# facebookresearch/GPU-DPF

Measured on AMD Instinct MI355X. Metric: DPFs/sec, higher is better.
Workload: dtype int32; 1 GPU; model=dpf-pir, entries=1048576, entry_size=16, prf=AES128, batch_per_gpu=512, global_batch=512, parallelism=dp1-replicated

## Files before the change

csrc/hip/dpf_hip_api.h:

```cpp
#pragma once
#include <cstddef>
#include <cstdint>

namespace gpudpf_hip {

void launch_fused(std::uintptr_t keys, std::uintptr_t table, std::uintptr_t out,
                  std::uintptr_t aes_tabs, int batch, long long n, int depth,
                  int zlog, int prf, std::uintptr_t stream,
                  std::uintptr_t scratch = 0, std::size_t scratch_bytes = 0,
                  int entry_words = 16);
std::size_t eval_scratch_bytes(int batch, int depth, int zlog);

void launch_fused_binned(std::uintptr_t keys, std::uintptr_t table,
                         std::uintptr_t bins, std::uintptr_t out,
                         std::uintptr_t aes_tabs, int batch, long long n,
                         int depth, int zlog, long long num_bins, int prf,
                         std::uintptr_t stream, std::uintptr_t scratch = 0,
                         std::size_t scratch_bytes = 0, int entry_words = 16);

int eval_slog(int batch, int depth, int zlog);
int eval_units_per_wg(int prf, int n_units, int entry_words = 16);

void launch_expand(std::uintptr_t keys, std::uintptr_t out,
                   std::uintptr_t aes_tabs, int batch, long long n, int depth,
                   int zlog, int prf, std::uintptr_t stream,
                   std::uintptr_t scratch = 0, std::size_t scratch_bytes = 0);

void launch_bfs(std::uintptr_t keys, std::uintptr_t out,
                std::uintptr_t aes_tabs, int batch, long long n, int depth,
                int prf, std::uintptr_t stream);

void launch_coop(std::uintptr_t keys, std::uintptr_t table, std::uintptr_t out,
                 std::uintptr_t aes_tabs, long long n, int depth, int zlog,
                 int prf, bool fused, std::uintptr_t stream);

void launch_naive(std::uintptr_t keys, std::uintptr_t out,
                  std::uintptr_t aes_tabs, int batch, long long n, int depth,
                  int prf, std::uintptr_t stream);

void launch_prf_sol(std::uintptr_t aes_tabs, std::uintptr_t out, int blocks,
                    int iters, int prf, std::uintptr_t stream);

void launch_probe_alu(std::uintptr_t a, std::uintptr_t b,
                      std::uintptr_t add_out, std::uintptr_t mul_out,
                      int count, std::uintptr_t stream);
void launch_probe_prf(std::uintptr_t seeds, std::uintptr_t aes_tabs,
                      std::uintptr_t pair0, std::uintptr_t pair1,
                      std::uintptr_t single0, std::uintptr_t single1,
                      std::uintptr_t low0, std::uintptr_t low1, int count,
                      int prf, std::uintptr_t stream);

struct KSplit;

KSplit gemm128_split(long long M, long long N, long long K);
void launch_gemm128(std::uintptr_t a, std::uintptr_t bt, std::uintptr_t c,
                    std::uintptr_t partials, std::size_t partials_bytes,
                    long long M, long long N, long long K,
                    std::uintptr_t stream);

KSplit gemm_u32_split(long long M, long long N, long long K);
void launch_digits(std::uintptr_t in, std::uintptr_t out, long long count,
                   std::uintptr_t stream);
void launch_gemm_u32_mfma(std::uintptr_t da, std::uintptr_t dbt,
                          std::uintptr_t c, long long M, long long N,
                          long long K, std::uintptr_t stream);

KSplit gemm_u32_stream_split(int batch, long long K, long long N);
void launch_gemm_u32_stream(std::uintptr_t a, std::uintptr_t b,
                            std::uintptr_t c, int batch, long long K,
                            long long N, std::uintptr_t stream);

}
```

csrc/hip/dpf_probes.hip:

```cpp

#include <hip/hip_runtime.h>

#include "dpf_hip_api.h"
#include "hip_util.h"
#include "prf_device.h"

namespace gpudpf_hip {

template <int PRF>
__global__ __launch_bounds__(PRF == PRF_AES128 ? 1024 : 256) void prf_sol_kernel(
    const u32* __restrict__ aes_tabs, u32* __restrict__ out, int iters) {
  extern __shared__ u32 smem[];
  const AesLds T = aes_lds_init<PRF>(smem, aes_tabs);
  uint4 seed = make_uint4(threadIdx.x + 1, blockIdx.x + 2, 3, 4);
  for (int i = 0; i < iters; ++i) {
    uint4 r0, r1;
    prf_pair<PRF>(seed, T, r0, r1);
    seed = make_uint4(r0.x ^ r1.x, r0.y ^ r1.y, r0.z ^ r1.z, r0.w ^ r1.w);
  }
  out[(u64)blockIdx.x * blockDim.x + threadIdx.x] = seed.x;
}

void launch_prf_sol(std::uintptr_t aes_tabs, std::uintptr_t out, int blocks,
                    int iters, int prf, std::uintptr_t stream) {
  const size_t shmem = aes_lds_u32(prf) * sizeof(u32);
  with_prf(prf, [&](auto P) {
    constexpr int PRF = decltype(P)::value;
    allow_large_lds((const void*)prf_sol_kernel<PRF>, shmem);
    const bool wide = PRF == PRF_AES128 && blocks % 4 == 0;
    hipLaunchKernelGGL(prf_sol_kernel<PRF>, dim3(wide ? blocks / 4 : blocks),
                       dim3(wide ? 1024 : 256), shmem, as_stream(stream),
                       as_ptr<const u32>(aes_tabs), as_ptr<u32>(out), iters);
  });
  HIP_CHECK(hipGetLastError());
}

__global__ __launch_bounds__(256) void probe_alu_kernel(
    const uint4* __restrict__ a, const uint4* __restrict__ b,
    uint4* __restrict__ add_out, uint4* __restrict__ mul_out, int count) {
  const int i = (int)(blockIdx.x * blockDim.x + threadIdx.x);
  if (i >= count) return;
  add_out[i] = add128(a[i], b[i]);
  const unsigned __int128 x =
      ((unsigned __int128)(((u64)a[i].w << 32) | a[i].z) << 64) |
      (((u64)a[i].y << 32) | a[i].x);
  const unsigned __int128 y =
      ((unsigned __int128)(((u64)b[i].w << 32) | b[i].z) << 64) |
      (((u64)b[i].y << 32) | b[i].x);
  const unsigned __int128 r = x * y;
  const u64 lo = (u64)r, hi = (u64)(r >> 64);
  mul_out[i] = make_uint4((u32)lo, (u32)(lo >> 32), (u32)hi, (u32)(hi >> 32));
}

template <int PRF>
__global__ __launch_bounds__(256) void probe_prf_kernel(
    const uint4* __restrict__ seeds, const u32* __restrict__ aes_tabs,
    uint4* __restrict__ pair0, uint4* __restrict__ pair1,
    uint4* __restrict__ single0, uint4* __restrict__ single1,
    u32* __restrict__ low0, u32* __restrict__ low1, int count) {
  extern __shared__ u32 smem[];
  const AesLds T = aes_lds_init<PRF>(smem, aes_tabs);
  const int i = (int)(blockIdx.x * blockDim.x + threadIdx.x);
  if (i >= count) return;
  const uint4 s = seeds[i];
  uint4 r0, r1;
  prf_pair<PRF>(s, T, r0, r1);
  pair0[i] = r0;
  pair1[i] = r1;
  single0[i] = prf_full<PRF>(s, 0, T);
  single1[i] = prf_full<PRF>(s, 1, T);
  u32 l0, l1;
  prf_pair_low<PRF>(s, T, l0, l1);
  low0[i] = l0;
  low1[i] = l1;
}

void launch_probe_alu(std::uintptr_t a, std::uintptr_t b,
                      std::uintptr_t add_out, std::uintptr_t mul_out,
                      int count, std::uintptr_t stream) {
  const int blocks = (count + 255) / 256;
  hipLaunchKernelGGL(probe_alu_kernel, dim3(blocks), dim3(256), 0,
                     as_stream(stream), as_ptr<const uint4>(a),
                     as_ptr<const uint4>(b), as_ptr<uint4>(add_out),
                     as_ptr<uint4>(mul_out), count);
  HIP_CHECK(hipGetLastError());
}

void launch_probe_prf(std::uintptr_t seeds, std::uintptr_t aes_tabs,
                      std::uintptr_t pair0, std::uintptr_t pair1,
                      std::uintptr_t single0, std::uintptr_t single1,
                      std::uintptr_t low0, std::uintptr_t low1, int count,
                      int prf, std::uintptr_t stream) {
  const int blocks = (count + 255) / 256;
  const size_t shmem = aes_lds_u32(prf) * sizeof(u32);
  with_prf(prf, [&](auto P) {
    constexpr int PRF = decltype(P)::value;
    allow_large_lds((const void*)probe_prf_kernel<PRF>, shmem);
    hipLaunchKernelGGL(probe_prf_kernel<PRF>, dim3(blocks), dim3(256), shmem,
                       as_stream(stream), as_ptr<const uint4>(seeds),
                       as_ptr<const u32>(aes_tabs), as_ptr<uint4>(pair0),
                       as_ptr<uint4>(pair1), as_ptr<uint4>(single0),
                       as_ptr<uint4>(single1), as_ptr<u32>(low0),
                       as_ptr<u32>(low1), count);
  });
  HIP_CHECK(hipGetLastError());
}

}
```

csrc/hip/hip_bindings.cc:

```cpp

#include <hip/hip_runtime.h>
#include <pybind11/pybind11.h>
#include <pybind11/stl.h>

#include <map>
#include <mutex>

#include "dpf_core.h"
#include "dpf_hip_api.h"
#include "hip_util.h"

namespace py = pybind11;

namespace {

std::mutex g_aes_mu;
std::map<int, void*> g_aes_tables;

std::uintptr_t ensure_aes_tables(int device) {
  std::lock_guard<std::mutex> lock(g_aes_mu);
  auto it = g_aes_tables.find(device);
  if (it != g_aes_tables.end()) return reinterpret_cast<std::uintptr_t>(it->second);
  gpudpf::u32 host[5 * 256];
  gpudpf::aes128_tables(host, host + 256, host + 512, host + 768, host + 1024);
  int prev = 0;
  HIP_CHECK(hipGetDevice(&prev));
  HIP_CHECK(hipSetDevice(device));
  void* dev = nullptr;
  HIP_CHECK(hipMalloc(&dev, sizeof(host)));
  HIP_CHECK(hipMemcpy(dev, host, sizeof(host), hipMemcpyHostToDevice));
  HIP_CHECK(hipSetDevice(prev));
  g_aes_tables[device] = dev;
  return reinterpret_cast<std::uintptr_t>(dev);
}

int device_count() {
  int n = 0;
  hipError_t e = hipGetDeviceCount(&n);
  if (e != hipSuccess) return 0;
  return n;
}

template <class... A>
auto split_tuple(gpudpf_hip::KSplit (*query)(A...)) {
  return [query](A... args) {
    const gpudpf_hip::KSplit s = query(args...);
    return std::make_pair(s.segs, s.kchunk);
  };
}

}

PYBIND11_MODULE(_hip, m) {
  m.doc() = "gpudpf MI355X HIP kernels (gfx950)";
  m.def("eval_fused", &gpudpf_hip::launch_fused, py::arg("keys"),
        py::arg("table"), py::arg("out"), py::arg("aes_tabs"), py::arg("batch"),
        py::arg("n"), py::arg("depth"), py::arg("zlog"), py::arg("prf"),
        py::arg("stream"), py::arg("scratch") = 0,
        py::arg("scratch_bytes") = 0, py::arg("entry_words") = 16,
        py::call_guard<py::gil_scoped_release>());
  m.def("eval_fused_binned", &gpudpf_hip::launch_fused_binned,
        py::arg("keys"), py::arg("table"), py::arg("bins"), py::arg("out"),
        py::arg("aes_tabs"), py::arg("batch"), py::arg("n"), py::arg("depth"),
        py::arg("zlog"), py::arg("num_bins"), py::arg("prf"),
        py::arg("stream"), py::arg("scratch") = 0,
        py::arg("scratch_bytes") = 0, py::arg("entry_words") = 16,
        py::call_guard<py::gil_scoped_release>());
  m.def("eval_scratch_bytes", &gpudpf_hip::eval_scratch_bytes,
        py::arg("batch"), py::arg("depth"), py::arg("zlog"));
  m.def("eval_slog", &gpudpf_hip::eval_slog, py::arg("batch"),
        py::arg("depth"), py::arg("zlog"));
  m.def("eval_units_per_wg", &gpudpf_hip::eval_units_per_wg, py::arg("prf"),
        py::arg("n_units"), py::arg("entry_words") = 16);
  m.def("eval_expand", &gpudpf_hip::launch_expand, py::arg("keys"),
        py::arg("out"), py::arg("aes_tabs"), py::arg("batch"), py::arg("n"),
        py::arg("depth"), py::arg("zlog"), py::arg("prf"), py::arg("stream"),
        py::arg("scratch") = 0, py::arg("scratch_bytes") = 0,
        py::call_guard<py::gil_scoped_release>());
  m.def("eval_bfs", &gpudpf_hip::launch_bfs, py::arg("keys"), py::arg("out"),
        py::arg("aes_tabs"), py::arg("batch"), py::arg("n"), py::arg("depth"),
        py::arg("prf"), py::arg("stream"),
        py::call_guard<py::gil_scoped_release>());
  m.def("eval_coop", &gpudpf_hip::launch_coop, py::arg("keys"),
        py::arg("table"), py::arg("out"), py::arg("aes_tabs"), py::arg("n"),
        py::arg("depth"), py::arg("zlog"), py::arg("prf"), py::arg("fused"),
        py::arg("stream"), py::call_guard<py::gil_scoped_release>());
  m.def("eval_naive", &gpudpf_hip::launch_naive, py::arg("keys"),
        py::arg("out"), py::arg("aes_tabs"), py::arg("batch"), py::arg("n"),
        py::arg("depth"), py::arg("prf"), py::arg("stream"),
        py::call_guard<py::gil_scoped_release>());
  m.def("gemm128", &gpudpf_hip::launch_gemm128, py::arg("a"), py::arg("bt"),
        py::arg("c"), py::arg("partials"), py::arg("partials_bytes"),
        py::arg("m"), py::arg("n"), py::arg("k"), py::arg("stream"),
        py::call_guard<py::gil_scoped_release>());
  m.def("gemm128_split", split_tuple(&gpudpf_hip::gemm128_split),
        py::arg("m"), py::arg("n"), py::arg("k"));
  m.def("prf_sol", &gpudpf_hip::launch_prf_sol, py::arg("aes_tabs"),
        py::arg("out"), py::arg("blocks"), py::arg("iters"), py::arg("prf"),
        py::arg("stream"), py::call_guard<py::gil_scoped_release>());
  m.def("digits", &gpudpf_hip::launch_digits, py::arg("inp"), py::arg("out"),
        py::arg("count"), py::arg("stream"),
        py::call_guard<py::gil_scoped_release>());
  m.def("gemm_u32_mfma", &gpudpf_hip::launch_gemm_u32_mfma, py::arg("da"),
        py::arg("dbt"), py::arg("c"), py::arg("m"), py::arg("n"), py::arg("k"),
        py::arg("stream"), py::call_guard<py::gil_scoped_release>());
  m.def("gemm_u32_split", split_tuple(&gpudpf_hip::gemm_u32_split),
        py::arg("m"), py::arg("n"), py::arg("k"));
  m.def("gemm_u32_stream", &gpudpf_hip::launch_gemm_u32_stream, py::arg("a"),
        py::arg("b"), py::arg("c"), py::arg("batch"), py::arg("k"),
        py::arg("n"), py::arg("stream"),
        py::call_guard<py::gil_scoped_release>());
  m.def("gemm_u32_stream_split",
        split_tuple(&gpudpf_hip::gemm_u32_stream_split), py::arg("batch"),
        py::arg("k"), py::arg("n"));
  m.def("probe_alu", &gpudpf_hip::launch_probe_alu, py::arg("a"), py::arg("b"),
        py::arg("add_out"), py::arg("mul_out"), py::arg("count"),
        py::arg("stream"), py::call_guard<py::gil_scoped_release>());
  m.def("probe_prf", &gpudpf_hip::launch_probe_prf, py::arg("seeds"),
        py::arg("aes_tabs"), py::arg("pair0"), py::arg("pair1"),
        py::arg("single0"), py::arg("single1"), py::arg("low0"),
        py::arg("low1"), py::arg("count"), py::arg("prf"), py::arg("stream"),
        py::call_guard<py::gil_scoped_release>());
  m.def("ensure_aes_tables", &ensure_aes_tables, py::arg("device"));
  m.def("device_count", &device_count);
}
```

csrc/hip/prf_device.h:

```cpp
#pragma once
#include "hip_util.h"

namespace gpudpf_hip {

__device__ __forceinline__ uint4 add128(uint4 a, uint4 b) {
  u64 alo = ((u64)a.y << 32) | a.x, ahi = ((u64)a.w << 32) | a.z;
  u64 blo = ((u64)b.y << 32) | b.x, bhi = ((u64)b.w << 32) | b.z;
  u64 lo = alo + blo;
  u64 hi = ahi + bhi + (lo < alo ? 1u : 0u);
  return make_uint4((u32)lo, (u32)(lo >> 32), (u32)hi, (u32)(hi >> 32));
}

__device__ __forceinline__ u32 rotl(u32 v, int s) {
  return (v << s) | (v >> (32 - s));
}
__device__ __forceinline__ u32 rotr8(u32 v) { return (v >> 8) | (v << 24); }
__device__ __forceinline__ u32 rotr16(u32 v) { return (v >> 16) | (v << 16); }
__device__ __forceinline__ u32 rotr24(u32 v) { return (v >> 24) | (v << 8); }

__device__ __forceinline__ uint4 key_root(const int* key) {
  const int* rp = key + kKeyRootInt;
  return make_uint4((u32)rp[0], (u32)rp[1], (u32)rp[2], (u32)rp[3]);
}

__device__ __forceinline__ uint4 prf_dummy_full(uint4 seed, u32 pos) {
  unsigned __int128 s =
      ((unsigned __int128)(((u64)seed.w << 32) | seed.z) << 64) |
      (((u64)seed.y << 32) | seed.x);
  unsigned __int128 m = (unsigned __int128)(pos + 4242u);
  unsigned __int128 r = s * m + m;
  u64 lo = (u64)r, hi = (u64)(r >> 64);
  return make_uint4((u32)lo, (u32)(lo >> 32), (u32)hi, (u32)(hi >> 32));
}

template <int N>
__device__ __forceinline__ void stream_init(u32 (&x)[16][N], int pos_w,
                                            const u32 (&init)[16]) {
#pragma unroll
  for (int w = 0; w < 16; ++w)
#pragma unroll
    for (int i = 0; i < N; ++i) x[w][i] = init[w] + (w == pos_w ? i : 0);
}

template <int N>
__device__ __forceinline__ uint4 stream_out(const u32 (&x)[16][N], int i,
                                            int lo, uint4 seed) {
  return make_uint4(x[lo][i] + seed.x, x[lo - 1][i] + seed.y,
                    x[lo - 2][i] + seed.z, x[lo - 3][i] + seed.w);
}

template <int PART = 4, int N>
__device__ __forceinline__ void salsa_qr(u32 (&x)[16][N], int a, int b, int c,
                                         int d) {
  auto step = [&](int t, int p, int q, int s) {
#pragma unroll
    for (int i = 0; i < N; ++i) x[t][i] ^= rotl(x[p][i] + x[q][i], s);
  };
  step(b, a, d, 7);
  if constexpr (PART > 1) step(c, b, a, 9);
  if constexpr (PART > 2) step(d, c, b, 13);
  if constexpr (PART > 3) step(a, d, c, 18);
}

template <bool LOW, int N>
__device__ __forceinline__ void salsa12(uint4 seed, u32 pos, u32 (&x)[16][N]) {
  stream_init(x, 9, {0x65787061u, seed.w, seed.z, seed.y, seed.x, 0x6e642033u,
                     0, 0, 0, pos, 0x322d6279u, 0, 0, 0, 0, 0x7465206bu});
#pragma unroll
  for (int r = 0; r < (LOW ? 5 : 6); ++r) {
    salsa_qr(x, 0, 4, 8, 12);
    salsa_qr(x, 5, 9, 13, 1);
    salsa_qr(x, 10, 14, 2, 6);
    salsa_qr(x, 15, 3, 7, 11);
    salsa_qr(x, 0, 1, 2, 3);
    salsa_qr(x, 5, 6, 7, 4);
    salsa_qr(x, 10, 11, 8, 9);
    salsa_qr(x, 15, 12, 13, 14);
  }
  if constexpr (LOW) {
    salsa_qr<1>(x, 0, 4, 8, 12);
    salsa_qr(x, 5, 9, 13, 1);
    salsa_qr<3>(x, 10, 14, 2, 6);
    salsa_qr<2>(x, 15, 3, 7, 11);
    salsa_qr<3>(x, 5, 6, 7, 4);
  }
}

__device__ __forceinline__ uint4 salsa12_core(uint4 seed, u32 pos) {
  u32 x[16][1];
  salsa12<false>(seed, pos, x);
  return stream_out(x, 0, 4, seed);
}

__device__ __forceinline__ void salsa12_pair_core(uint4 seed, uint4& r0,
                                                  uint4& r1) {
  u32 x[16][2];
  salsa12<false>(seed, 0, x);
  r0 = stream_out(x, 0, 4, seed);
  r1 = stream_out(x, 1, 4, seed);
}

__device__ __forceinline__ void salsa12_pair_low_core(uint4 seed, u32& lo0,
                                                      u32& lo1) {
  u32 x[16][2];
  salsa12<true>(seed, 0, x);
  lo0 = x[4][0] + seed.x;
  lo1 = x[4][1] + seed.x;
}

template <int PART = 8, int N>
__device__ __forceinline__ void chacha_qr(u32 (&x)[16][N], int a, int b, int c,
                                          int d) {
  static_assert(PART >= 6 && PART <= 8, "only the tail is ever pruned");
  auto add = [&](int t, int s) {
#pragma unroll
    for (int i = 0; i < N; ++i) x[t][i] += x[s][i];
  };
  auto xor_rotl = [&](int t, int s, int r) {
#pragma unroll
    for (int i = 0; i < N; ++i) x[t][i] ^= x[s][i];
#pragma unroll
    for (int i = 0; i < N; ++i) x[t][i] = rotl(x[t][i], r);
  };
  add(a, b);  xor_rotl(d, a, 16);
  add(c, d);  xor_rotl(b, c, 12);
  add(a, b);  xor_rotl(d, a, 8);
  if constexpr (PART > 6) add(c, d);
  if constexpr (PART > 7) xor_rotl(b, c, 7);
}

template <bool LOW, int N>
__device__ __forceinline__ void chacha12(uint4 seed, u32 pos,
                                         u32 (&x)[16][N]) {
  stream_init(x, 13, {0x65787061u, 0x6e642033u, 0x322d6279u, 0x7465206bu,
                      seed.w, seed.z, seed.y, seed.x, 0, 0, 0, 0, 0, pos, 0, 0});
#pragma unroll
  for (int r = 0; r < (LOW ? 5 : 6); ++r) {
    chacha_qr(x, 0, 4, 8, 12);
    chacha_qr(x, 1, 5, 9, 13);
    chacha_qr(x, 2, 6, 10, 14);
    chacha_qr(x, 3, 7, 11, 15);
    chacha_qr(x, 0, 5, 10, 15);
    chacha_qr(x, 1, 6, 11, 12);
    chacha_qr(x, 2, 7, 8, 13);
    chacha_qr(x, 3, 4, 9, 14);
  }
  if constexpr (LOW) {
    chacha_qr<7>(x, 0, 4, 8, 12);
    chacha_qr<6>(x, 1, 5, 9, 13);
    chacha_qr(x, 2, 6, 10, 14);
    chacha_qr(x, 3, 7, 11, 15);
    chacha_qr(x, 2, 7, 8, 13);
  }
}

__device__ __forceinline__ uint4 chacha12_core(uint4 seed, u32 pos) {
  u32 x[16][1];
  chacha12<false>(seed, pos, x);
  return stream_out(x, 0, 7, seed);
}

__device__ __forceinline__ void chacha12_pair_core(uint4 seed, uint4& r0,
                                                   uint4& r1) {
  u32 x[16][2];
  chacha12<false>(seed, 0, x);
  r0 = stream_out(x, 0, 7, seed);
  r1 = stream_out(x, 1, 7, seed);
}

__device__ __forceinline__ void chacha12_pair_low_core(uint4 seed, u32& lo0,
                                                       u32& lo1) {
  u32 x[16][2];
  chacha12<true>(seed, 0, x);
  lo0 = x[7][0] + seed.x;
  lo1 = x[7][1] + seed.x;
}

constexpr int AES_REP = 64;
constexpr int AES_LDS_WORDS = 256 * AES_REP;

__host__ __device__ constexpr int aes_lds_u32(int prf) {
  return prf == PRF_AES128 ? AES_LDS_WORDS : 0;
}

__device__ __forceinline__ u32 xor3(u32 a, u32 b, u32 c) {
  return __builtin_amdgcn_bitop3_b32(a, b, c, 0x96);
}

__device__ __forceinline__ u32 aes_sb_hi(u32 ta, u32 tb) {
  return __builtin_amdgcn_perm(ta, tb, 0x06020c0cu);
}
__device__ __forceinline__ u32 aes_sb_lo(u32 tc, u32 td) {
  return __builtin_amdgcn_perm(tc, td, 0x0c0c0602u);
}

struct AesLds {
  u32 lane4;
  static __device__ __forceinline__ AesLds lane() {
    return AesLds{((u32)threadIdx.x & 63u) << 2};
  }
  typedef __attribute__((address_space(3))) const u32 lds_u32;
  static __device__ __forceinline__ u32 ld(u32 byte_addr) {
    return *reinterpret_cast<lds_u32*>(byte_addr);
  }
  template <int K>
  __device__ __forceinline__ u32 addr_b(u32 w) const {
    return __builtin_amdgcn_perm(w, lane4, 0x0c0c0000u | ((4u + K) << 8));
  }
  template <int K>
  __device__ __forceinline__ u32 te0_b(u32 w) const { return ld(addr_b<K>(w)); }
  __device__ __forceinline__ u32 col(u32 a, u32 b, u32 c, u32 d, u32 k) const {
    return xor3(xor3(te0_b<3>(a), rotr8(te0_b<2>(b)), rotr16(te0_b<1>(c))),
                rotr24(te0_b<0>(d)), k);
  }
  __device__ __forceinline__ u32 last(u32 a, u32 b, u32 c, u32 d, u32 k) const {
    return xor3(aes_sb_hi(te0_b<3>(a), te0_b<2>(b)),
                aes_sb_lo(te0_b<1>(c), te0_b<0>(d)), k);
  }
};

template <int PRF>
__device__ __forceinline__ void aes_stage_table(
    u32* lds0, const u32* __restrict__ aes_tabs) {
  if constexpr (PRF == PRF_AES128) {
    for (int idx = (int)threadIdx.x; idx < AES_LDS_WORDS;
         idx += (int)blockDim.x)
      lds0[idx] = aes_tabs[idx >> 6];
  }
}

template <int PRF>
__device__ __forceinline__ AesLds aes_lds_init(
    u32* lds0, const u32* __restrict__ aes_tabs) {
  aes_stage_table<PRF>(lds0, aes_tabs);
  if constexpr (PRF == PRF_AES128) __syncthreads();
  return AesLds::lane();
}

template <bool LOW>
__device__ __forceinline__ void aes_cipher_pair(uint4 seed, const AesLds& T,
                                                uint4& ra, uint4& rb) {
  u32 k0 = __builtin_bswap32(seed.x), k1 = __builtin_bswap32(seed.y),
      k2 = __builtin_bswap32(seed.z), k3 = __builtin_bswap32(seed.w);
  u32 s0 = k0, s1 = k1, s2 = k2, s3 = k3;
  u32 u0 = (1u << 24) ^ k0, u1 = k1, u2 = k2, u3 = k3;
  u32 rcon = 0x01u;
  auto next_round_key = [&] {
    k0 = xor3(aes_sb_hi(T.te0_b<2>(k3), T.te0_b<1>(k3)),
              aes_sb_lo(T.te0_b<0>(k3), T.te0_b<3>(k3)), k0) ^ (rcon << 24);
    rcon = (rcon << 1) ^ ((rcon & 0x80u) ? 0x11bu : 0u);
    rcon &= 0xffu;
    k1 ^= k0; k2 ^= k1; k3 ^= k2;
  };
  int r_begin = 1;
#ifndef GPUDPF_AES_NOSHARE
  {
    const u32 t33 = T.te0_b<3>(s3), t32 = T.te0_b<2>(s3),
              t31 = T.te0_b<1>(s3), t30 = T.te0_b<0>(s3);
    k0 = xor3(aes_sb_hi(t32, t31), aes_sb_lo(t30, t33), k0) ^ (rcon << 24);
    rcon = 0x02u;
    k1 ^= k0; k2 ^= k1; k3 ^= k2;
    const u32 a0 = T.addr_b<3>(s0);
    const u32 A = AesLds::ld(a0);
    u32 n0 = xor3(xor3(A, rotr8(T.te0_b<2>(s1)), rotr16(T.te0_b<1>(s2))),
                  rotr24(t30), k0);
    u32 n1 = xor3(xor3(T.te0_b<3>(s1), rotr8(T.te0_b<2>(s2)), rotr16(t31)),
                  rotr24(T.te0_b<0>(s0)), k1);
    u32 n2 = xor3(xor3(T.te0_b<3>(s2), rotr8(t32), rotr16(T.te0_b<1>(s0))),
                  rotr24(T.te0_b<0>(s1)), k2);
    u32 n3 = xor3(xor3(t33, rotr8(T.te0_b<2>(s0)), rotr16(T.te0_b<1>(s1))),
                  rotr24(T.te0_b<0>(s2)), k3);
    const u32 m0 = xor3(n0, A, AesLds::ld(a0 ^ 256u));
    next_round_key();
    const u32 c0 = xor3(rotr8(T.te0_b<2>(n1)), rotr16(T.te0_b<1>(n2)),
                        rotr24(T.te0_b<0>(n3))) ^ k0;
    const u32 c1 = xor3(T.te0_b<3>(n1), rotr8(T.te0_b<2>(n2)),
                        rotr16(T.te0_b<1>(n3))) ^ k1;
    const u32 c2 = xor3(T.te0_b<3>(n2), rotr8(T.te0_b<2>(n3)),
                        rotr24(T.te0_b<0>(n1))) ^ k2;
    const u32 c3 = xor3(T.te0_b<3>(n3), rotr16(T.te0_b<1>(n1)),
                        rotr24(T.te0_b<0>(n2))) ^ k3;
    s0 = T.te0_b<3>(n0) ^ c0;
    u0 = T.te0_b<3>(m0) ^ c0;
    s1 = rotr24(T.te0_b<0>(n0)) ^ c1;
    u1 = rotr24(T.te0_b<0>(m0)) ^ c1;
    s2 = rotr16(T.te0_b<1>(n0)) ^ c2;
    u2 = rotr16(T.te0_b<1>(m0)) ^ c2;
    s3 = rotr8(T.te0_b<2>(n0)) ^ c3;
    u3 = rotr8(T.te0_b<2>(m0)) ^ c3;
    r_begin = 3;
  }
#endif
#pragma unroll
  for (int r = r_begin; r < 10; ++r) {
    next_round_key();
    u32 n0 = T.col(s0, s1, s2, s3, k0);
    u32 m0 = T.col(u0, u1, u2, u3, k0);
    u32 n1 = T.col(s1, s2, s3, s0, k1);
    u32 m1 = T.col(u1, u2, u3, u0, k1);
    u32 n2 = T.col(s2, s3, s0, s1, k2);
    u32 m2 = T.col(u2, u3, u0, u1, k2);
    u32 n3 = T.col(s3, s0, s1, s2, k3);
    u32 m3 = T.col(u3, u0, u1, u2, k3);
    s0 = n0; s1 = n1; s2 = n2; s3 = n3;
    u0 = m0; u1 = m1; u2 = m2; u3 = m3;
  }
  next_round_key();
  u32 o0 = T.last(s0, s1, s2, s3, k0);
  u32 p0 = T.last(u0, u1, u2, u3, k0);
  if constexpr (LOW) {
    ra = make_uint4(__builtin_bswap32(o0), 0, 0, 0);
    rb = make_uint4(__builtin_bswap32(p0), 0, 0, 0);
    return;
  }
  u32 o1 = T.last(s1, s2, s3, s0, k1);
  u32 p1 = T.last(u1, u2, u3, u0, k1);
  u32 o2 = T.last(s2, s3, s0, s1, k2);
  u32 p2 = T.last(u2, u3, u0, u1, k2);
  u32 o3 = T.last(s3, s0, s1, s2, k3);
  u32 p3 = T.last(u3, u0, u1, u2, k3);
  ra = make_uint4(__builtin_bswap32(o0), __builtin_bswap32(o1),
                  __builtin_bswap32(o2), __builtin_bswap32(o3));
  rb = make_uint4(__builtin_bswap32(p0), __builtin_bswap32(p1),
                  __builtin_bswap32(p2), __builtin_bswap32(p3));
}

template <int PRF>
__device__ __forceinline__ uint4 prf_full(uint4 seed, u32 pos,
                                          const AesLds& T) {
  if constexpr (PRF == PRF_DUMMY) return prf_dummy_full(seed, pos);
  if constexpr (PRF == PRF_SALSA20) return salsa12_core(seed, pos);
  if constexpr (PRF == PRF_CHACHA20) return chacha12_core(seed, pos);
  if constexpr (PRF == PRF_AES128) {
    uint4 a, b;
    aes_cipher_pair<false>(seed, T, a, b);
    return pos ? b : a;
  }
}

template <int PRF>
__device__ __forceinline__ void prf_pair(uint4 seed, const AesLds& T,
                                         uint4& r0, uint4& r1) {
  if constexpr (PRF == PRF_AES128) {
    aes_cipher_pair<false>(seed, T, r0, r1);
  } else if constexpr (PRF == PRF_SALSA20) {
    salsa12_pair_core(seed, r0, r1);
  } else if constexpr (PRF == PRF_CHACHA20) {
    chacha12_pair_core(seed, r0, r1);
  } else {
    r0 = prf_full<PRF>(seed, 0, T);
    r1 = prf_full<PRF>(seed, 1, T);
  }
}

template <int PRF>
__device__ __forceinline__ void prf_pair_low(uint4 seed, const AesLds& T,
                                             u32& r0, u32& r1) {
  if constexpr (PRF == PRF_DUMMY) {
    r0 = seed.x * 4242u + 4242u;
    r1 = seed.x * 4243u + 4243u;
  } else if constexpr (PRF == PRF_SALSA20) {
    salsa12_pair_low_core(seed, r0, r1);
  } else if constexpr (PRF == PRF_CHACHA20) {
    chacha12_pair_low_core(seed, r0, r1);
  } else {
    uint4 a, b;
    aes_cipher_pair<true>(seed, T, a, b);
    r0 = a.x;
    r1 = b.x;
  }
}

}
```

Before: 33020 dpfs/s.

## Use Te0/Te2 LDS tables with rotated state to cut AES rotates

Restructures the AES T-table round. LDS now holds 32 lane-replicated copies each of Te0 and Te2 (Te0 rotated by 16) instead of 64 copies of Te0 alone. State and round keys are kept in a byte-rotated representation, so each column mix needs only one rotate, applied after the XORs, rather than three separate rotates. The first round is also peeled and merged with the shared-seed path. This aims to lower VALU instruction count per round, at the cost of halving the per-lane table replication, which could increase LDS bank conflicts.

```diff
diff --git a/csrc/hip/dpf_hip_api.h b/csrc/hip/dpf_hip_api.h
--- a/csrc/hip/dpf_hip_api.h
+++ b/csrc/hip/dpf_hip_api.h
@@ -49,6 +49,8 @@
                       std::uintptr_t single0, std::uintptr_t single1,
                       std::uintptr_t low0, std::uintptr_t low1, int count,
                       int prf, std::uintptr_t stream);
+void launch_probe_aes_lds(std::uintptr_t aes_tabs, std::uintptr_t out,
+                          int threads, std::uintptr_t stream);
 
 struct KSplit;
 
diff --git a/csrc/hip/dpf_probes.hip b/csrc/hip/dpf_probes.hip
--- a/csrc/hip/dpf_probes.hip
+++ b/csrc/hip/dpf_probes.hip
@@ -75,6 +75,28 @@
   low1[i] = l1;
 }
 
+__global__ __launch_bounds__(1024) void probe_aes_lds_kernel(
+    const u32* __restrict__ aes_tabs, u32* __restrict__ out) {
+  extern __shared__ u32 smem[];
+  aes_lds_init<PRF_AES128>(smem, aes_tabs);
+  for (int idx = (int)threadIdx.x; idx < AES_LDS_WORDS; idx += (int)blockDim.x)
+    out[idx] = smem[idx];
+}
+
+void launch_probe_aes_lds(std::uintptr_t aes_tabs, std::uintptr_t out,
+                          int threads, std::uintptr_t stream) {
+  if (threads < 64 || threads > 1024 || threads % 64 != 0)
+    throw std::invalid_argument(
+        "probe_aes_lds: threads must be a multiple of 64 in [64, 1024]");
+  check_ptrs("probe_aes_lds", {aes_tabs, out});
+  const size_t shmem = aes_lds_u32(PRF_AES128) * sizeof(u32);
+  allow_large_lds((const void*)probe_aes_lds_kernel, shmem);
+  hipLaunchKernelGGL(probe_aes_lds_kernel, dim3(1), dim3(threads), shmem,
+                     as_stream(stream), as_ptr<const u32>(aes_tabs),
+                     as_ptr<u32>(out));
+  HIP_CHECK(hipGetLastError());
+}
+
 void launch_probe_alu(std::uintptr_t a, std::uintptr_t b,
                       std::uintptr_t add_out, std::uintptr_t mul_out,
                       int count, std::uintptr_t stream) {
diff --git a/csrc/hip/hip_bindings.cc b/csrc/hip/hip_bindings.cc
--- a/csrc/hip/hip_bindings.cc
+++ b/csrc/hip/hip_bindings.cc
@@ -121,6 +121,9 @@
         py::arg("single0"), py::arg("single1"), py::arg("low0"),
         py::arg("low1"), py::arg("count"), py::arg("prf"), py::arg("stream"),
         py::call_guard<py::gil_scoped_release>());
+  m.def("probe_aes_lds", &gpudpf_hip::launch_probe_aes_lds,
+        py::arg("aes_tabs"), py::arg("out"), py::arg("threads"),
+        py::arg("stream"), py::call_guard<py::gil_scoped_release>());
   m.def("ensure_aes_tables", &ensure_aes_tables, py::arg("device"));
   m.def("device_count", &device_count);
 }
diff --git a/csrc/hip/prf_device.h b/csrc/hip/prf_device.h
--- a/csrc/hip/prf_device.h
+++ b/csrc/hip/prf_device.h
@@ -15,8 +15,6 @@
   return (v << s) | (v >> (32 - s));
 }
 __device__ __forceinline__ u32 rotr8(u32 v) { return (v >> 8) | (v << 24); }
-__device__ __forceinline__ u32 rotr16(u32 v) { return (v >> 16) | (v << 16); }
-__device__ __forceinline__ u32 rotr24(u32 v) { return (v >> 24) | (v << 8); }
 
 __device__ __forceinline__ uint4 key_root(const int* key) {
   const int* rp = key + kKeyRootInt;
@@ -176,8 +174,10 @@
   lo1 = x[7][1] + seed.x;
 }
 
-constexpr int AES_REP = 64;
+constexpr int AES_COPIES = 32;
+constexpr int AES_REP = AES_COPIES * 2;
 constexpr int AES_LDS_WORDS = 256 * AES_REP;
+constexpr u32 AES_TE2_BYTES = AES_COPIES * 4;
 
 __host__ __device__ constexpr int aes_lds_u32(int prf) {
   return prf == PRF_AES128 ? AES_LDS_WORDS : 0;
@@ -187,35 +187,61 @@
   return __builtin_amdgcn_bitop3_b32(a, b, c, 0x96);
 }
 
-__device__ __forceinline__ u32 aes_sb_hi(u32 ta, u32 tb) {
-  return __builtin_amdgcn_perm(ta, tb, 0x06020c0cu);
-}
-__device__ __forceinline__ u32 aes_sb_lo(u32 tc, u32 td) {
-  return __builtin_amdgcn_perm(tc, td, 0x0c0c0602u);
+template <int PA, int PB, int BA = 2, int BB = 2>
+__device__ __forceinline__ u32 aes_sb_pair(u32 ta, u32 tb) {
+  static_assert(PA != PB, "the two bytes land in different places");
+  constexpr u32 sel = (0x0c0c0c0cu & ~(0xffu << (8 * PA)) &
+                       ~(0xffu << (8 * PB))) |
+                      ((4u + BA) << (8 * PA)) | ((u32)BB << (8 * PB));
+  return __builtin_amdgcn_perm(ta, tb, sel);
+}
+
+__device__ __forceinline__ u32 bswap_rol8(u32 x) {
+  return __builtin_amdgcn_perm(0u, x, 0x01020300u);
 }
 
 struct AesLds {
   u32 lane4;
   static __device__ __forceinline__ AesLds lane() {
-    return AesLds{((u32)threadIdx.x & 63u) << 2};
+    return AesLds{((u32)threadIdx.x & (u32)(AES_COPIES - 1)) << 2};
   }
   typedef __attribute__((address_space(3))) const u32 lds_u32;
   static __device__ __forceinline__ u32 ld(u32 byte_addr) {
     return *reinterpret_cast<lds_u32*>(byte_addr);
   }
+  static __device__ __forceinline__ u32 ld_te2(u32 byte_addr) {
+    return reinterpret_cast<lds_u32*>(byte_addr)[AES_TE2_BYTES / 4];
+  }
   template <int K>
   __device__ __forceinline__ u32 addr_b(u32 w) const {
     return __builtin_amdgcn_perm(w, lane4, 0x0c0c0000u | ((4u + K) << 8));
   }
   template <int K>
   __device__ __forceinline__ u32 te0_b(u32 w) const { return ld(addr_b<K>(w)); }
-  __device__ __forceinline__ u32 col(u32 a, u32 b, u32 c, u32 d, u32 k) const {
-    return xor3(xor3(te0_b<3>(a), rotr8(te0_b<2>(b)), rotr16(te0_b<1>(c))),
-                rotr24(te0_b<0>(d)), k);
-  }
-  __device__ __forceinline__ u32 last(u32 a, u32 b, u32 c, u32 d, u32 k) const {
-    return xor3(aes_sb_hi(te0_b<3>(a), te0_b<2>(b)),
-                aes_sb_lo(te0_b<1>(c), te0_b<0>(d)), k);
+  template <int K>
+  __device__ __forceinline__ u32 te2_b(u32 w) const {
+    return ld_te2(addr_b<K>(w));
+  }
+  template <int K>
+  __device__ __forceinline__ u32 addr_kb(u32 q) const {
+    return addr_b<(K + 1) & 3>(q);
+  }
+  template <int K>
+  __device__ __forceinline__ u32 te0_kb(u32 q) const { return ld(addr_kb<K>(q)); }
+  template <int K>
+  __device__ __forceinline__ u32 te2_kb(u32 q) const {
+    return ld_te2(addr_kb<K>(q));
+  }
+  static __device__ __forceinline__ u32 mix(u32 te0a, u32 te0b, u32 te2c,
+                                            u32 te2d, u32 q) {
+    return xor3(te0a, te2c, rotr8(xor3(te0b, te2d, q)));
+  }
+  __device__ __forceinline__ u32 col(u32 a, u32 b, u32 c, u32 d, u32 q) const {
+    return mix(te0_b<3>(a), te0_b<2>(b), te2_b<1>(c), te2_b<0>(d), q);
+  }
+  __device__ __forceinline__ u32 last(u32 a, u32 b, u32 c, u32 d, u32 q) const {
+    return xor3(aes_sb_pair<0, 3>(te0_b<3>(a), te0_b<2>(b)),
+                aes_sb_pair<2, 1>(te0_b<1>(c), te0_b<0>(d)), q);
   }
 };
 
@@ -225,7 +251,7 @@
   if constexpr (PRF == PRF_AES128) {
     for (int idx = (int)threadIdx.x; idx < AES_LDS_WORDS;
          idx += (int)blockDim.x)
-      lds0[idx] = aes_tabs[idx >> 6];
+      lds0[idx] = aes_tabs[(((idx >> 5) & 1) << 9) + (idx >> 6)];
   }
 }
 
@@ -240,89 +266,89 @@
 template <bool LOW>
 __device__ __forceinline__ void aes_cipher_pair(uint4 seed, const AesLds& T,
                                                 uint4& ra, uint4& rb) {
-  u32 k0 = __builtin_bswap32(seed.x), k1 = __builtin_bswap32(seed.y),
-      k2 = __builtin_bswap32(seed.z), k3 = __builtin_bswap32(seed.w);
-  u32 s0 = k0, s1 = k1, s2 = k2, s3 = k3;
-  u32 u0 = (1u << 24) ^ k0, u1 = k1, u2 = k2, u3 = k3;
-  u32 rcon = 0x01u;
+  u32 q0 = bswap_rol8(seed.x), q1 = bswap_rol8(seed.y),
+      q2 = bswap_rol8(seed.z), q3 = bswap_rol8(seed.w);
+  u32 rcon = 0x02u;
   auto next_round_key = [&] {
-    k0 = xor3(aes_sb_hi(T.te0_b<2>(k3), T.te0_b<1>(k3)),
-              aes_sb_lo(T.te0_b<0>(k3), T.te0_b<3>(k3)), k0) ^ (rcon << 24);
+    q0 = xor3(aes_sb_pair<3, 2>(T.te0_b<2>(q3), T.te0_b<1>(q3)),
+              aes_sb_pair<1, 0>(T.te0_b<0>(q3), T.te0_b<3>(q3)), q0) ^ rcon;
     rcon = (rcon << 1) ^ ((rcon & 0x80u) ? 0x11bu : 0u);
     rcon &= 0xffu;
-    k1 ^= k0; k2 ^= k1; k3 ^= k2;
+    q1 ^= q0; q2 ^= q1; q3 ^= q2;
   };
-  int r_begin = 1;
+  const u32 a0 = T.addr_kb<3>(q0);
+  const u32 x03 = AesLds::ld(a0), x02 = T.te0_kb<2>(q0),
+            x01 = T.te2_kb<1>(q0), x00 = T.te2_kb<0>(q0);
+  const u32 x13 = T.te0_kb<3>(q1), x12 = T.te0_kb<2>(q1),
+            x11 = T.te2_kb<1>(q1), x10 = T.te2_kb<0>(q1);
+  const u32 x23 = T.te0_kb<3>(q2), x22 = T.te0_kb<2>(q2),
+            x21 = T.te2_kb<1>(q2), x20 = T.te2_kb<0>(q2);
+  const u32 x33 = T.te0_kb<3>(q3), x32 = T.te0_kb<2>(q3),
+            x31 = T.te2_kb<1>(q3), x30 = T.te2_kb<0>(q3);
+  const u32 x03b = AesLds::ld(a0 ^ 256u);
+  q0 = xor3(aes_sb_pair<3, 2, 0, 0>(x31, x30), aes_sb_pair<1, 0>(x33, x32),
+            q0) ^ 0x01u;
+  q1 ^= q0; q2 ^= q1; q3 ^= q2;
+  u32 s0 = AesLds::mix(x03, x12, x21, x30, q0);
+  u32 s1 = AesLds::mix(x13, x22, x31, x00, q1);
+  u32 s2 = AesLds::mix(x23, x32, x01, x10, q2);
+  u32 s3 = AesLds::mix(x33, x02, x11, x20, q3);
+  u32 u0 = xor3(s0, x03, x03b), u1 = s1, u2 = s2, u3 = s3;
+  int r_begin = 2;
 #ifndef GPUDPF_AES_NOSHARE
   {
-    const u32 t33 = T.te0_b<3>(s3), t32 = T.te0_b<2>(s3),
-              t31 = T.te0_b<1>(s3), t30 = T.te0_b<0>(s3);
-    k0 = xor3(aes_sb_hi(t32, t31), aes_sb_lo(t30, t33), k0) ^ (rcon << 24);
-    rcon = 0x02u;
-    k1 ^= k0; k2 ^= k1; k3 ^= k2;
-    const u32 a0 = T.addr_b<3>(s0);
-    const u32 A = AesLds::ld(a0);
-    u32 n0 = xor3(xor3(A, rotr8(T.te0_b<2>(s1)), rotr16(T.te0_b<1>(s2))),
-                  rotr24(t30), k0);
-    u32 n1 = xor3(xor3(T.te0_b<3>(s1), rotr8(T.te0_b<2>(s2)), rotr16(t31)),
-                  rotr24(T.te0_b<0>(s0)), k1);
-    u32 n2 = xor3(xor3(T.te0_b<3>(s2), rotr8(t32), rotr16(T.te0_b<1>(s0))),
-                  rotr24(T.te0_b<0>(s1)), k2);
-    u32 n3 = xor3(xor3(t33, rotr8(T.te0_b<2>(s0)), rotr16(T.te0_b<1>(s1))),
-                  rotr24(T.te0_b<0>(s2)), k3);
-    const u32 m0 = xor3(n0, A, AesLds::ld(a0 ^ 256u));
+    const u32 n0 = s0, n1 = s1, n2 = s2, n3 = s3, m0 = u0;
     next_round_key();
-    const u32 c0 = xor3(rotr8(T.te0_b<2>(n1)), rotr16(T.te0_b<1>(n2)),
-                        rotr24(T.te0_b<0>(n3))) ^ k0;
-    const u32 c1 = xor3(T.te0_b<3>(n1), rotr8(T.te0_b<2>(n2)),
-                        rotr16(T.te0_b<1>(n3))) ^ k1;
-    const u32 c2 = xor3(T.te0_b<3>(n2), rotr8(T.te0_b<2>(n3)),
-                        rotr24(T.te0_b<0>(n1))) ^ k2;
-    const u32 c3 = xor3(T.te0_b<3>(n3), rotr16(T.te0_b<1>(n1)),
-                        rotr24(T.te0_b<0>(n2))) ^ k3;
-    s0 = T.te0_b<3>(n0) ^ c0;
-    u0 = T.te0_b<3>(m0) ^ c0;
-    s1 = rotr24(T.te0_b<0>(n0)) ^ c1;
-    u1 = rotr24(T.te0_b<0>(m0)) ^ c1;
-    s2 = rotr16(T.te0_b<1>(n0)) ^ c2;
-    u2 = rotr16(T.te0_b<1>(m0)) ^ c2;
-    s3 = rotr8(T.te0_b<2>(n0)) ^ c3;
-    u3 = rotr8(T.te0_b<2>(m0)) ^ c3;
+    const u32 e13 = T.te0_b<3>(n1), e12 = T.te0_b<2>(n1),
+              e11 = T.te2_b<1>(n1), e10 = T.te2_b<0>(n1);
+    const u32 e23 = T.te0_b<3>(n2), e22 = T.te0_b<2>(n2),
+              e21 = T.te2_b<1>(n2), e20 = T.te2_b<0>(n2);
+    const u32 e33 = T.te0_b<3>(n3), e32 = T.te0_b<2>(n3),
+              e31 = T.te2_b<1>(n3), e30 = T.te2_b<0>(n3);
+    const u32 r0 = rotr8(xor3(e12, e30, q0));
+    s0 = xor3(T.te0_b<3>(n0), e21, r0);
+    u0 = xor3(T.te0_b<3>(m0), e21, r0);
+    s1 = AesLds::mix(e13, e22, e31, T.te2_b<0>(n0), q1);
+    u1 = AesLds::mix(e13, e22, e31, T.te2_b<0>(m0), q1);
+    s2 = AesLds::mix(e23, e32, T.te2_b<1>(n0), e10, q2);
+    u2 = AesLds::mix(e23, e32, T.te2_b<1>(m0), e10, q2);
+    s3 = AesLds::mix(e33, T.te0_b<2>(n0), e11, e20, q3);
+    u3 = AesLds::mix(e33, T.te0_b<2>(m0), e11, e20, q3);
     r_begin = 3;
   }
 #endif
 #pragma unroll
   for (int r = r_begin; r < 10; ++r) {
     next_round_key();
-    u32 n0 = T.col(s0, s1, s2, s3, k0);
-    u32 m0 = T.col(u0, u1, u2, u3, k0);
-    u32 n1 = T.col(s1, s2, s3, s0, k1);
-    u32 m1 = T.col(u1, u2, u3, u0, k1);
-    u32 n2 = T.col(s2, s3, s0, s1, k2);
-    u32 m2 = T.col(u2, u3, u0, u1, k2);
-    u32 n3 = T.col(s3, s0, s1, s2, k3);
-    u32 m3 = T.col(u3, u0, u1, u2, k3);
+    u32 n0 = T.col(s0, s1, s2, s3, q0);
+    u32 m0 = T.col(u0, u1, u2, u3, q0);
+    u32 n1 = T.col(s1, s2, s3, s0, q1);
+    u32 m1 = T.col(u1, u2, u3, u0, q1);
+    u32 n2 = T.col(s2, s3, s0, s1, q2);
+    u32 m2 = T.col(u2, u3, u0, u1, q2);
+    u32 n3 = T.col(s3, s0, s1, s2, q3);
+    u32 m3 = T.col(u3, u0, u1, u2, q3);
     s0 = n0; s1 = n1; s2 = n2; s3 = n3;
     u0 = m0; u1 = m1; u2 = m2; u3 = m3;
   }
   next_round_key();
-  u32 o0 = T.last(s0, s1, s2, s3, k0);
-  u32 p0 = T.last(u0, u1, u2, u3, k0);
+  u32 o0 = T.last(s0, s1, s2, s3, q0);
+  u32 p0 = T.last(u0, u1, u2, u3, q0);
   if constexpr (LOW) {
-    ra = make_uint4(__builtin_bswap32(o0), 0, 0, 0);
-    rb = make_uint4(__builtin_bswap32(p0), 0, 0, 0);
+    ra = make_uint4(bswap_rol8(o0), 0, 0, 0);
+    rb = make_uint4(bswap_rol8(p0), 0, 0, 0);
     return;
   }
-  u32 o1 = T.last(s1, s2, s3, s0, k1);
-  u32 p1 = T.last(u1, u2, u3, u0, k1);
-  u32 o2 = T.last(s2, s3, s0, s1, k2);
-  u32 p2 = T.last(u2, u3, u0, u1, k2);
-  u32 o3 = T.last(s3, s0, s1, s2, k3);
-  u32 p3 = T.last(u3, u0, u1, u2, k3);
-  ra = make_uint4(__builtin_bswap32(o0), __builtin_bswap32(o1),
-                  __builtin_bswap32(o2), __builtin_bswap32(o3));
-  rb = make_uint4(__builtin_bswap32(p0), __builtin_bswap32(p1),
-                  __builtin_bswap32(p2), __builtin_bswap32(p3));
+  u32 o1 = T.last(s1, s2, s3, s0, q1);
+  u32 p1 = T.last(u1, u2, u3, u0, q1);
+  u32 o2 = T.last(s2, s3, s0, s1, q2);
+  u32 p2 = T.last(u2, u3, u0, u1, q2);
+  u32 o3 = T.last(s3, s0, s1, s2, q3);
+  u32 p3 = T.last(u3, u0, u1, u2, q3);
+  ra = make_uint4(bswap_rol8(o0), bswap_rol8(o1), bswap_rol8(o2),
+                  bswap_rol8(o3));
+  rb = make_uint4(bswap_rol8(p0), bswap_rol8(p1), bswap_rol8(p2),
+                  bswap_rol8(p3));
 }
 
 template <int PRF>
```

Result: faster. 37690 dpfs/s, median of 6 (+14.1%).
